# Arlo0o/StereoScene

Hardware: AMD Instinct MI355X
Metric: voxels/sec fwd+bwd, 256x256x32 grid D=192 (higher is better)
Workload: dtype f32; 1 GPU; kitti_d192: stereo pair features 2x[B,640,48,160] -> 256x256x32 occupancy, D=192, fwd+bwd incl. 4 losses; batch_per_gpu=1, global_batch=1, parallelism=dp1, train_mode=True

## Files before the change

### stereoscene_amd/csrc/conv_mfma.hip

```cpp
#include "common.h"
#include "conv_bf16.h"
#include "conv_thin_mfma.h"

#include <algorithm>
#include <cstdio>
#include <vector>
#include <array>
#include <map>
#include <mutex>
#include <type_traits>

namespace {

typedef float f32x16 __attribute__((ext_vector_type(16)));

struct ConvGeom {
  int B, Cin, Cout, CinPad, CoutPad;
  int Di, Hi, Wi, Do, Ho, Wo;
  int kd, kh, kw, sd, sh, sw, pd, ph, pw, dd, dh, dw;
  int form;
  int relu, accumulate;
  int hint;
  int chunk_taps;
  int bf16;
// ... 452 lines not shown
      if (khi >= g.kh || kwi >= g.kw) continue;
      const int tap = (kdi * g.kh + khi) * g.kw + kwi;
      float* dst = ws + (((size_t)chunk_id * taps + tap) * g.Cq) * g.Cp;
#pragma unroll
      for (int a = 0; a < MQ; ++a)
#pragma unroll
        for (int e = 0; e < MP; ++e)
#pragma unroll
          for (int r = 0; r < 16; ++r) {
            const int row = (qt * MQ + a) * 32 + (r & 3) + 8 * (r >> 2) + 4 * lk;
            if (row < g.Cq && pok[e]) dst[(size_t)row * g.Cp + poff[e]] = acc[a][e][c][t][r];
          }
    }
}

__global__ void __launch_bounds__(256)
wgrad_reduce_kernel(const float* __restrict__ ws, float* __restrict__ gw, int nchunks, int taps, int Cq, int Cp,
                    long total, long cstride) {
  __shared__ float part[8][33];
  const int e = threadIdx.x & 31, row = threadIdx.x >> 5;
  const long i = (long)blockIdx.x * 32 + e;
  float s = 0.0f;
  if (i < total)
    for (int c = row; c < nchunks; c += 8) s += ws[(size_t)c * cstride + i];
  part[row][e] = s;
  __syncthreads();
  if (row == 0 && i < total) {
    float t = 0.0f;
#pragma unroll
    for (int r = 0; r < 8; ++r) t += part[r][e];
    const int p = (int)(i % Cp);
    const int q = (int)((i / Cp) % Cq);
    const int tap = (int)(i / ((long)Cp * Cq));
    gw[((size_t)p * Cq + q) * taps + tap] = t;
  }
}

__global__ void __launch_bounds__(256)
wgrad_reduce_tiled_kernel(const float* __restrict__ ws, float* __restrict__ gw, int nchunks, int taps, int Cq, int Cp,
                          long total, long cstride) {
  extern __shared__ float tile[];
  const int P = 8 * taps + 1;
  const int e = threadIdx.x & 31, row = threadIdx.x >> 5;
  const int p0 = blockIdx.x * 32, q0 = blockIdx.y * 8;
  const bool ok = p0 + e < Cp && q0 + row < Cq;
  for (int tap = 0; tap < taps; ++tap) {
    float s = 0.0f;
    if (ok) {
      const float* src = ws + ((size_t)tap * Cq + q0 + row) * Cp + p0 + e;
#pragma unroll 4
      for (int c = 0; c < nchunks; ++c) s += src[(size_t)c * cstride];
    }
    tile[e * P + row * taps + tap] = s;
  }
  __syncthreads();
  const int run = 8 * taps;
  for (int j = threadIdx.x; j < 32 * run; j += 256) {
    const int pe = j / run, r = j - pe * run;
    const int q = q0 + r / taps, tap = r % taps, pp = p0 + pe;
    if (pp < Cp && q < Cq) gw[((size_t)pp * Cq + q) * taps + tap] = tile[pe * P + r];
  }
}

typedef float wr_f4 __attribute__((ext_vector_type(4)));
__global__ void __launch_bounds__(256)
wgrad_reduce_stage_kernel(float* __restrict__ ws, int nchunks, int per, long total4) {
  const long j = (long)blockIdx.x * 256 + threadIdx.x;
  if (j >= total4) return;
  const int c0 = blockIdx.y * per, c1 = min(nchunks, c0 + per);
  wr_f4* base = reinterpret_cast<wr_f4*>(ws) + (size_t)c0 * total4 + j;
  const wr_f4* p = base;
  wr_f4 a[8];
#pragma unroll
  for (int u = 0; u < 8; ++u) a[u] = wr_f4{0.0f, 0.0f, 0.0f, 0.0f};
  for (int c = c0; c < c1; c += 8) {
#pragma unroll
    for (int u = 0; u < 8; ++u)
      if (c + u < c1) a[u] += p[(size_t)u * total4];
    p += 8 * total4;
  }
  *base = ((a[0] + a[1]) + (a[2] + a[3])) + ((a[4] + a[5]) + (a[6] + a[7]));
}

void launch_wgrad_reduce(float* partial, float* gw, int nchunks, int taps, int Cq, int Cp, hipStream_t st) {
  const long total = (long)taps * Cq * Cp;
  long cstride = total;
  static const int two_stage = ssbev_tune("SSBEV_WGRAD_REDUCE2") ? atoi(ssbev_tune("SSBEV_WGRAD_REDUCE2")) : 1;
  if (two_stage && nchunks >= 64 && total % 4 == 0) {
    const long total4 = total / 4, bx = cdiv(total4, 256);
    int nsl = (int)std::min<long>(std::max<long>(cdiv(2048, bx), 1), nchunks / 8);
    const int per = cdiv(nchunks, nsl);
    nsl = cdiv(nchunks, per);
    hipLaunchKernelGGL(wgrad_reduce_stage_kernel, dim3((unsigned)bx, (unsigned)nsl), dim3(256), 0, st, partial, nchunks, per,
                       total4);
    nchunks = nsl;
    cstride = (long)per * total;
  }
  if (taps <= 32 && (long)cdiv(Cp, 32) * cdiv(Cq, 8) >= 128) {
    hipLaunchKernelGGL(wgrad_reduce_tiled_kernel, dim3(cdiv(Cp, 32), cdiv(Cq, 8)), dim3(256),
                       (size_t)32 * (8 * taps + 1) * sizeof(float), st, partial, gw, nchunks, taps, Cq, Cp, total, cstride);
  } else {
    hipLaunchKernelGGL(wgrad_reduce_kernel, dim3(cdiv(total, 32)), dim3(256), 0, st, partial, gw, nchunks, taps, Cq, Cp,
                       total, cstride);
  }
}

bool conv_dims_ok(const ssbev_conv_dims* d) {
  if (!d) return false;
  if (d->B <= 0 || d->Cin <= 0 || d->Cout <= 0) return false;
  if (d->Di <= 0 || d->Hi <= 0 || d->Wi <= 0 || d->Do <= 0 || d->Ho <= 0 || d->Wo <= 0) return false;
  if (d->kd <= 0 || d->kh <= 0 || d->kw <= 0 || d->sd <= 0 || d->sh <= 0 || d->sw <= 0) return false;
  if (d->dd <= 0 || d->dh <= 0 || d->dw <= 0 || d->pd < 0 || d->ph < 0 || d->pw < 0) return false;
  if (d->kd > 8 || d->kh > 8 || d->kw > 8) return false;
  const bool strided = d->sd > 1 || d->sh > 1 || d->sw > 1;
  const bool dilated = d->dd > 1 || d->dh > 1 || d->dw > 1;
  if (strided && dilated) return false;
  return true;
}

int pad8(int c) { return (c + 7) & ~7; }
int pad32(int c) { return (c + 31) & ~31; }
size_t align256b(size_t x) { return (x + 255) & ~(size_t)255; }

bool is_k3_p1_d1(const ssbev_conv_dims* d, int s) {
  return d->kd == 3 && d->kh == 3 && d->kw == 3 && d->sd == s && d->sh == s && d->sw == s &&
         d->pd == 1 && d->ph == 1 && d->pw == 1 && d->dd == 1 && d->dh == 1 && d->dw == 1;
}
bool same_grid(const ssbev_conv_dims* d) { return d->Di == d->Do && d->Hi == d->Ho && d->Wi == d->Wo; }

ConvGeom make_gather_geom(const ssbev_conv_dims* d, int mode) {
  const bool fwd = mode == 0;
  ConvGeom g;
  g.B = d->B; g.Cin = fwd ? d->Cin : d->Cout; g.Cout = fwd ? d->Cout : d->Cin; g.CinPad = pad8(g.Cin); g.CoutPad = pad32(g.Cout);
  g.Di = fwd ? d->Di : d->Do; g.Hi = fwd ? d->Hi : d->Ho; g.Wi = fwd ? d->Wi : d->Wo;
  g.Do = fwd ? d->Do : d->Di; g.Ho = fwd ? d->Ho : d->Hi; g.Wo = fwd ? d->Wo : d->Wi;
  g.kd = d->kd; g.kh = d->kh; g.kw = d->kw; g.sd = d->sd; g.sh = d->sh; g.sw = d->sw;
  g.pd = d->pd; g.ph = d->ph; g.pw = d->pw; g.dd = d->dd; g.dh = d->dh; g.dw = d->dw;
  g.form = (d->transposed != 0) == fwd ? 1 : 0;
  g.relu = fwd ? d->relu : 0; g.accumulate = d->accumulate;
  g.hint = d->tile_hint >= 10 ? d->tile_hint : 0;
  g.chunk_taps = 0; g.bf16 = d->precision == 1;
  return g;
}

template <int MT, int NT, int QU>
int launch_gather(const float* x, const float* wp, const float* bias, float* y, const ConvGeom& g, hipStream_t st) {
  long Mtot = (long)g.B * g.Do * g.Ho * g.Wo;
  int classes = 1;
  if (g.form == 1) {
    classes = g.sd * g.sh * g.sw;
    Mtot = (long)g.B * ((g.Do + g.sd - 1) / g.sd) * ((g.Ho + g.sh - 1) / g.sh) * ((g.Wo + g.sw - 1) / g.sw);
  }
  dim3 grid(cdiv(Mtot, 4 * MT * 32), cdiv(g.Cout, NT * 32), classes), block(256);
  constexpr bool PIPE = NT == 5;
  if (g.bf16) {
    constexpr int QB = QU < 2 ? 2 : QU;
    if ((g.CinPad >> 3) % QB == 0)
      hipLaunchKernelGGL((conv_gather_kernel<MT, NT, QB, 4, false, PIPE, true>), grid, block, 0, st, x, wp, bias, y, g);
    else if ((g.CinPad >> 3) % 2 == 0)
      hipLaunchKernelGGL((conv_gather_kernel<MT, NT, 2, 4, false, PIPE, true>), grid, block, 0, st, x, wp, bias, y, g);
    else
      hipLaunchKernelGGL((conv_gather_kernel<MT, NT, 1, 4, false, false, true>), grid, block, 0, st, x, wp, bias, y, g);
    return ssbev_launch_status();
  }
  if ((g.CinPad >> 3) % QU == 0)
    hipLaunchKernelGGL((conv_gather_kernel<MT, NT, QU, 4, false, PIPE>), grid, block, 0, st, x, wp, bias, y, g);
  else
    hipLaunchKernelGGL((conv_gather_kernel<MT, NT, 1, 4, false, PIPE>), grid, block, 0, st, x, wp, bias, y, g);
  return ssbev_launch_status();
}

template <int MT, int QU>
int launch_gather_ldsb(const float* x, const float* wp, const float* bias, float* y, const ConvGeom& g, hipStream_t st) {
  constexpr int WPB = 16;
  long Mtot = (long)g.B * g.Do * g.Ho * g.Wo;
  int classes = 1;
  if (g.form == 1) {
    classes = g.sd * g.sh * g.sw;
    Mtot = (long)g.B * ((g.Do + g.sd - 1) / g.sd) * ((g.Ho + g.sh - 1) / g.sh) * ((g.Wo + g.sw - 1) / g.sw);
  }
  const size_t per_tap = (size_t)(g.CinPad >> 3) * 2 * 32 * 16;
  const int taps_total = g.kd * g.kh * g.kw;
  int chunk = (int)((144 * 1024) / per_tap);
  if (chunk < 1) return SSBEV_EINVAL;
  if (chunk > taps_total) chunk = taps_total;
  const int passes = (taps_total + chunk - 1) / chunk;
  chunk = (taps_total + passes - 1) / passes;
  ConvGeom gg = g;
  gg.chunk_taps = chunk;
  const size_t lds = per_tap * chunk;
  auto kern = g.bf16 ? conv_gather_kernel<MT, 1, QU, WPB, true, false, true> : conv_gather_kernel<MT, 1, QU, WPB, true>;
  if (lds > 64 * 1024 && hipFuncSetAttribute(reinterpret_cast<const void*>(kern),
                                              hipFuncAttributeMaxDynamicSharedMemorySize, (int)lds) != hipSuccess)
    return SSBEV_ELAUNCH;
  dim3 grid(cdiv(Mtot, WPB * MT * 32), cdiv(g.Cout, 32), classes), block(WPB * 64);
  hipLaunchKernelGGL(kern, grid, block, lds, st, x, wp, bias, y, gg);
  return ssbev_launch_status();
}

template <int MT, int NT>
int launch_gather_qu(int qu, const float* x, const float* wp, const float* bias, float* y, const ConvGeom& g,
                     hipStream_t st) {
  if (qu == 4) return launch_gather<MT, NT, 4>(x, wp, bias, y, g, st);
  if (qu == 2) return launch_gather<MT, NT, 2>(x, wp, bias, y, g, st);
  return launch_gather<MT, NT, 1>(x, wp, bias, y, g, st);
}

int launch_gather_cfg(int mt, int nt, int qu, const float* x, const float* wp, const float* bias, float* y,
                      const ConvGeom& g, hipStream_t st) {
  switch (mt * 10 + nt) {
    case 41: return launch_gather_qu<4, 1>(qu, x, wp, bias, y, g, st);
    case 21: return launch_gather_qu<2, 1>(qu, x, wp, bias, y, g, st);
    case 11: return launch_gather_qu<1, 1>(qu, x, wp, bias, y, g, st);
    case 24: return launch_gather_qu<2, 4>(qu, x, wp, bias, y, g, st);
    case 22: return launch_gather_qu<2, 2>(qu, x, wp, bias, y, g, st);
    case 12: return launch_gather_qu<1, 2>(qu, x, wp, bias, y, g, st);
    case 15: return launch_gather_qu<1, 5>(qu, x, wp, bias, y, g, st);
    case 14: return launch_gather_qu<1, 4>(qu, x, wp, bias, y, g, st);
    case 31: return launch_gather_qu<3, 1>(qu, x, wp, bias, y, g, st);
    case 23: return launch_gather_qu<2, 3>(qu, x, wp, bias, y, g, st);
    case 26: return launch_gather_qu<2, 6>(qu, x, wp, bias, y, g, st);
    case 16: return launch_gather_qu<1, 6>(qu, x, wp, bias, y, g, st);
    case 13: return launch_gather_qu<1, 3>(qu, x, wp, bias, y, g, st);
    case 91: return launch_gather_ldsb<2, 2>(x, wp, bias, y, g, st);
    case 92: return launch_gather_ldsb<1, 2>(x, wp, bias, y, g, st);
    default: return SSBEV_EINVAL;
  }
}

long gather_blocks(const ConvGeom& g, int MT, int NT) {
  long M = (long)g.B * g.Do * g.Ho * g.Wo;
  long classes = 1;
  if (g.form == 1) {
    classes = (long)g.sd * g.sh * g.sw;
    M = (long)g.B * ((g.Do + g.sd - 1) / g.sd) * ((g.Ho + g.sh - 1) / g.sh) * ((g.Wo + g.sw - 1) / g.sw);
  }
  return ((M + 4 * MT * 32 - 1) / (4 * MT * 32)) * ((g.Cout + NT * 32 - 1) / (NT * 32)) * classes;
}

__device__ const float kGatherZeros[4] __attribute__((aligned(16))) = {0.f, 0.f, 0.f, 0.f};

template <int WN, int MW, int WGN>
__global__ void __launch_bounds__(256, 2)
conv_igemm_kernel(const float* __restrict__ x, const float* __restrict__ wp, const float* __restrict__ bias,
                  float* __restrict__ y, ConvGeom g, int mblocks, int nblocks) {
  constexpr int WGM = 4 / WGN;
  constexpr int BM = 32 * MW * WGM, BN = 32 * WN * WGN, BK = 32;
  constexpr int AF = BM * BK, BF = BK * BN, SF = AF + BF;
  constexpr int AI = AF / 256, BI = BF / 256;
  constexpr int AE = (AI + 3) / 4, BE = (BI + 3) / 4;
  extern __shared__ __align__(16) float lds[];
  long* t_src = reinterpret_cast<long*>(lds + 2 * SF);
  long* t_dst = t_src + BM;
  unsigned* t_msk = reinterpret_cast<unsigned*>(t_dst + BM);
  const int tid = threadIdx.x, lane = tid & 63, wave = __builtin_amdgcn_readfirstlane(tid >> 6);
  const int li = lane & 31, lk = lane >> 5;
  const int wm = wave / WGN, wn = wave % WGN;

  int par_d = 0, par_h = 0, par_w = 0;
  int Dc = g.Do, Hc = g.Ho, Wc = g.Wo;
  if (g.form == 1) {
    int cls = (int)gridDim.z - 1 - (int)blockIdx.z;
    par_w = cls % g.sw; cls /= g.sw;
    par_h = cls % g.sh; cls /= g.sh;
    par_d = cls;
    Dc = (g.Do - par_d + g.sd - 1) / g.sd; Hc = (g.Ho - par_h + g.sh - 1) / g.sh; Wc = (g.Wo - par_w + g.sw - 1) / g.sw;
  }
  const long Mtot = (long)g.B * Dc * Hc * Wc;
  int mb, nb;
  {
    const unsigned n = gridDim.x, L = blockIdx.x;
    const unsigned xcd = L & 7, q = n >> 3, r = n & 7;
    const unsigned base = xcd < r ? xcd * (q + 1) : r * (q + 1) + (xcd - r) * q;
    const unsigned Lp = base + (L >> 3);
    nb = (int)(Lp % (unsigned)nblocks);
    mb = (int)(Lp / (unsigned)nblocks);
  }
  const long m0 = (long)mb * BM;
  const int n0 = nb * BN;
  if (m0 >= Mtot) return;

  int kd0 = 0, kh0 = 0, kw0 = 0, kds = 1, khs = 1, kws = 1;
  if (g.form == 1) {
    kd0 = (par_d + g.pd) % g.sd; kh0 = (par_h + g.ph) % g.sh; kw0 = (par_w + g.pw) % g.sw;
    kds = g.sd; khs = g.sh; kws = g.sw;
  }
  const int nkd = (g.kd - kd0 + kds - 1) / kds, nkh = (g.kh - kh0 + khs - 1) / khs, nkw = (g.kw - kw0 + kws - 1) / kws;
  const int ntaps = (kd0 < g.kd && kh0 < g.kh && kw0 < g.kw) ? nkd * nkh * nkw : 0;
  int step_d, step_h, step_w;
  if (g.form == 0) { step_d = g.dd; step_h = g.dh; step_w = g.dw; }
  else { step_d = -(kds * g.dd) / g.sd; step_h = -(khs * g.dh) / g.sh; step_w = -(kws * g.dw) / g.sw; }

  if (tid < BM) {
    long m = m0 + tid;
    const bool ok = m < Mtot;
    if (!ok) m = 0;
    const int ow = (int)(m % Wc); m /= Wc;
    const int oh = (int)(m % Hc); m /= Hc;
    const int od = (int)(m % Dc);
    const int ob = (int)(m / Dc);
    int bd, bh, bw;
    if (g.form == 0) {
      bd = od * g.sd - g.pd; bh = oh * g.sh - g.ph; bw = ow * g.sw - g.pw;
    } else {
      bd = od + (par_d + g.pd - kd0 * g.dd) / g.sd;
      bh = oh + (par_h + g.ph - kh0 * g.dh) / g.sh;
      bw = ow + (par_w + g.pw - kw0 * g.dw) / g.sw;
    }
    unsigned msk = 0;
    for (int i = 0; i < nkd && i < 8; ++i) { const int v = bd + i * step_d; msk |= (v >= 0 && v < g.Di) ? (1u << i) : 0u; }
    for (int i = 0; i < nkh && i < 8; ++i) { const int v = bh + i * step_h; msk |= (v >= 0 && v < g.Hi) ? (1u << (8 + i)) : 0u; }
    for (int i = 0; i < nkw && i < 8; ++i) { const int v = bw + i * step_w; msk |= (v >= 0 && v < g.Wi) ? (1u << (16 + i)) : 0u; }
    t_msk[tid] = ok ? msk : 0u;
    t_src[tid] = ((((long)ob * g.Di + bd) * g.Hi + bh) * g.Wi + bw) * (long)g.Cin;
    long dst;
    if (g.form == 0) dst = (((long)ob * g.Do + od) * g.Ho + oh) * g.Wo + ow;
    else dst = (((long)ob * g.Do + (od * g.sd + par_d)) * g.Ho + (oh * g.sh + par_h)) * g.Wo + (ow * g.sw + par_w);
    t_dst[tid] = ok ? dst * (long)g.Cout : -1;
  }
  __syncthreads();

  const float* ap[AE]; unsigned am[AE];
#pragma unroll
  for (int e = 0; e < AE; ++e) {
    const int item = (wave + 4 * e) * 64 + lane, row = item >> 3, slot = item & 7;
    const bool on = wave + 4 * e < AI;
    ap[e] = x + (on ? t_src[row] : 0) + ((slot ^ ((row >> 1) & 7)) << 2);
    am[e] = on ? t_msk[row] : 0u;
  }
  const int Q = g.CinPad >> 3;
  long boff[BE];
#pragma unroll
  for (int e = 0; e < BE; ++e) {
    const int j = wave + 4 * e, f = j * 256 + 4 * lane;
    const int r8 = f / (BN * 4), col = f % (BN * 4);
    boff[e] = n0 + col / 4 < g.CoutPad ? (long)r8 * g.CoutPad * 4 + (long)n0 * 4 + col : -1;
  }
  const int cq_n = g.Cin >> 5;
  const int nst = ntaps * cq_n;
  int i_ia = 0, i_ib = 0, i_ic = 0, i_cq = 0;
  auto issue = [&](int buf) {
    const int tap = ((kd0 + i_ia * kds) * g.kh + (kh0 + i_ib * khs)) * g.kw + (kw0 + i_ic * kws);
    const long toff = (((long)i_ia * step_d * g.Hi + (long)i_ib * step_h) * g.Wi + (long)i_ic * step_w) * g.Cin + i_cq * 32;
    const unsigned need = (1u << i_ia) | (1u << (8 + i_ib)) | (1u << (16 + i_ic));
#pragma unroll
    for (int e = 0; e < AE; ++e) {
      if (AI % 4 != 0 && wave + 4 * e >= AI) break;
      const float* src = ((am[e] & need) == need) ? ap[e] + toff : kGatherZeros;
      __builtin_amdgcn_global_load_lds(src, lds + buf * SF + (wave + 4 * e) * 256, 16, 0, 0);
    }
    const float* wb = wp + ((size_t)tap * Q + 4 * i_cq) * 2 * g.CoutPad * 4;
#pragma unroll
    for (int e = 0; e < BE; ++e) {
      if (BI % 4 != 0 && wave + 4 * e >= BI) break;
      const float* bsrc = boff[e] >= 0 ? wb + boff[e] : kGatherZeros;
      __builtin_amdgcn_global_load_lds(bsrc, lds + buf * SF + AF + (wave + 4 * e) * 256, 16, 0, 0);
    }
    if (++i_cq == cq_n) {
      i_cq = 0;
      if (++i_ic == nkw) { i_ic = 0; if (++i_ib == nkh) { i_ib = 0; ++i_ia; } }
    }
  };

  f32x16 acc[MW][WN];
#pragma unroll
  for (int mt = 0; mt < MW; ++mt)
#pragma unroll
    for (int nt = 0; nt < WN; ++nt)
#pragma unroll
      for (int r = 0; r < 16; ++r) acc[mt][nt][r] = 0.0f;

  typedef float v4f __attribute__((ext_vector_type(4)));
  if (nst > 0) issue(0);
  for (int st = 0; st < nst; ++st) {
    const int buf = st & 1;
    asm volatile("s_waitcnt vmcnt(0)" ::: "memory");
    __builtin_amdgcn_s_barrier();
    if (st + 1 < nst) issue(buf ^ 1);
    const float* as = lds + buf * SF;
    const float* bs = as + AF;
    v4f ac[MW], bc[WN], an[MW], bn[WN];
    auto fetch = [&](int q, v4f (&a)[MW], v4f (&bf)[WN]) {
#pragma unroll
      for (int mt = 0; mt < MW; ++mt) {
        const int row = (wm * MW + mt) * 32 + li;
        a[mt] = *reinterpret_cast<const v4f*>(as + row * BK + (((2 * q + lk) ^ ((row >> 1) & 7)) << 2));
      }
#pragma unroll
      for (int nt = 0; nt < WN; ++nt)
        bf[nt] = *reinterpret_cast<const v4f*>(bs + ((2 * q + lk) * BN + (wn * WN + nt) * 32 + li) * 4);
    };
    fetch(0, ac, bc);
#pragma unroll
    for (int q = 0; q < BK / 8; ++q) {
      if (q + 1 < BK / 8) fetch(q + 1, an, bn);
      __builtin_amdgcn_sched_barrier(0);
#pragma unroll
      for (int t = 0; t < 4; ++t)
#pragma unroll
        for (int mt = 0; mt < MW; ++mt)
#pragma unroll
          for (int nt = 0; nt < WN; ++nt)
            acc[mt][nt] = __builtin_amdgcn_mfma_f32_32x32x2f32(ac[mt][t], bc[nt][t], acc[mt][nt], 0, 0, 0);
#pragma unroll
      for (int mt = 0; mt < MW; ++mt) ac[mt] = an[mt];
#pragma unroll
      for (int nt = 0; nt < WN; ++nt) bc[nt] = bn[nt];
    }
    asm volatile("s_waitcnt lgkmcnt(0)" ::: "memory");
  }

  float bv[WN];
#pragma unroll
  for (int nt = 0; nt < WN; ++nt) {
    const int co = min(n0 + (wn * WN + nt) * 32 + li, g.Cout - 1);
    bv[nt] = bias ? bias[co] : 0.0f;
  }
  long rowbase[MW][16];
#pragma unroll
  for (int mt = 0; mt < MW; ++mt)
#pragma unroll
    for (int r = 0; r < 16; ++r) rowbase[mt][r] = t_dst[(wm * MW + mt) * 32 + (r & 3) + 8 * (r >> 2) + 4 * lk];
  if (g.accumulate) {
#pragma unroll
    for (int mt = 0; mt < MW; ++mt)
#pragma unroll
      for (int r0 = 0; r0 < 16; r0 += 8) {
        float oldv[8][WN];
#pragma unroll
        for (int r = 0; r < 8; ++r)
#pragma unroll
          for (int nt = 0; nt < WN; ++nt) {
            const int co = n0 + (wn * WN + nt) * 32 + li;
            oldv[r][nt] = (rowbase[mt][r0 + r] >= 0 && co < g.Cout) ? y[rowbase[mt][r0 + r] + co] : 0.0f;
          }
#pragma unroll
        for (int r = 0; r < 8; ++r)
#pragma unroll
          for (int nt = 0; nt < WN; ++nt) acc[mt][nt][r0 + r] += oldv[r][nt];
      }
  }
#pragma unroll
  for (int nt = 0; nt < WN; ++nt) asm volatile("" : "+v"(bv[nt]));
#pragma unroll
  for (int nt = 0; nt < WN; ++nt) {
    const int co = n0 + (wn * WN + nt) * 32 + li;
    if (co >= g.Cout) continue;
#pragma unroll
    for (int mt = 0; mt < MW; ++mt)
#pragma unroll
      for (int r = 0; r < 16; ++r) {
        if (rowbase[mt][r] >= 0) {
          float v = acc[mt][nt][r] + bv[nt];
          if (g.relu) v = fmaxf(v, 0.0f);
          y[rowbase[mt][r] + co] = v;
        }
      }
  }
}

bool conv_igemm_applicable(const ConvGeom& g) {
  const char* env = ssbev_env("SSBEV_IGEMM");
  const int mode = env ? atoi(env) : 2;
  if (mode == 0 || g.bf16 || g.hint) return false;
  if (g.Cin % 32 != 0 || g.Cout % 4 != 0 || g.Cout < 64) return false;
  if (g.kd > 8 || g.kh > 8 || g.kw > 8) return false;
  const int taps = g.kd * g.kh * g.kw;
  if (taps == 1) return false;
  if (g.form == 0 && g.sd * g.sh * g.sw == 1 && mode != 2)
    return false;
  const long M = (long)g.B * g.Do * g.Ho * g.Wo;
  return M >= 2048;
}

template <int WN, int MW, int WGN>
int launch_igemm_t(const float* x, const float* wp, const float* bias, float* y, const ConvGeom& g, hipStream_t st) {
  constexpr int BM = 32 * MW * (4 / WGN), BN = 32 * WN * WGN;
  long Mtot = (long)g.B * g.Do * g.Ho * g.Wo;
  int classes = 1;
  if (g.form == 1) {
    classes = g.sd * g.sh * g.sw;
    Mtot = (long)g.B * ((g.Do + g.sd - 1) / g.sd) * ((g.Ho + g.sh - 1) / g.sh) * ((g.Wo + g.sw - 1) / g.sw);
  }
  const int mblocks = (int)((Mtot + BM - 1) / BM), nblocks = (g.Cout + BN - 1) / BN;
  const size_t lds = (size_t)2 * (BM * 32 + 32 * BN) * sizeof(float) + (size_t)BM * (2 * sizeof(long) + sizeof(unsigned));
  auto kern = conv_igemm_kernel<WN, MW, WGN>;
  if (hipFuncSetAttribute(reinterpret_cast<const void*>(kern), hipFuncAttributeMaxDynamicSharedMemorySize, (int)lds) != hipSuccess)
    return SSBEV_ELAUNCH;
  hipLaunchKernelGGL(kern, dim3((unsigned)(mblocks * nblocks), 1, classes), dim3(256), lds, st, x, wp, bias, y, g, mblocks, nblocks);
  return ssbev_launch_status();
}

int launch_igemm(const float* x, const float* wp, const float* bias, float* y, const ConvGeom& g, hipStream_t st) {
  long Mtot = (long)g.B * g.Do * g.Ho * g.Wo;
  long classes = 1;
  if (g.form == 1) {
    classes = (long)g.sd * g.sh * g.sw;
    Mtot = (long)g.B * ((g.Do + g.sd - 1) / g.sd) * ((g.Ho + g.sh - 1) / g.sh) * ((g.Wo + g.sw - 1) / g.sw);
  }
  const int force = ssbev_tune("SSBEV_IGEMM_TILE") ? atoi(ssbev_tune("SSBEV_IGEMM_TILE")) : 0;
  const bool wide = g.CoutPad % 128 == 0;
  const long need = g.form == 1 ? 1024 : 512;
  const int cand[3][2] = {{128, wide ? 128 : 64}, {64, wide ? 128 : 64}, {64, 64}};
  int bm = 64, bn = 64;
  for (int i = 0; i < 3; ++i) {
    const long blocks = ((Mtot + cand[i][0] - 1) / cand[i][0]) * ((g.Cout + cand[i][1] - 1) / cand[i][1]) * classes;
    if (blocks >= need) { bm = cand[i][0]; bn = cand[i][1]; break; }
  }
  if (force) { bm = force / 1000; bn = force % 1000; }
  if (bm == 128 && bn == 128) return launch_igemm_t<2, 2, 2>(x, wp, bias, y, g, st);
  if (bm == 128 && bn == 64) return launch_igemm_t<1, 2, 2>(x, wp, bias, y, g, st);
  if (bm == 64 && bn == 128) return launch_igemm_t<2, 1, 2>(x, wp, bias, y, g, st);
  if (bm == 64 && bn == 64) return launch_igemm_t<1, 1, 2>(x, wp, bias, y, g, st);
  return SSBEV_EINVAL;
}

int dispatch_gather(const float* x, const float* wp, const float* bias, float* y, const ConvGeom& g, hipStream_t st) {
  if (g.hint) return launch_gather_cfg(g.hint / 100, (g.hint / 10) % 10, g.hint % 10, x, wp, bias, y, g, st);
  const long Mtot = (long)g.B * g.Do * g.Ho * g.Wo;
  if (Mtot <= 8192 && g.Cout % 160 == 0 && g.Cout >= 640 && g.sd * g.sh * g.sw == 1)
    return launch_gather_cfg(1, 5, 4, x, wp, bias, y, g, st);
  {
    const long classes = g.form == 1 ? (long)g.sd * g.sh * g.sw : 1;
    const long keff = g.form == 1 ? (long)cdiv(g.kd, g.sd) * cdiv(g.kh, g.sh) * cdiv(g.kw, g.sw) * g.Cin
                                  : (long)g.kd * g.kh * g.kw * g.Cin;
    if (Mtot / classes <= 8192 && keff <= 8192 && g.Cout > 64)
      return launch_gather_cfg(1, 1, g.form == 1 ? 1 : 4, x, wp, bias, y, g, st);
  }
  {
    const size_t wbytes = (size_t)g.kd * g.kh * g.kw * (g.CinPad >> 3) * 2 * 32 * 16;
    if (g.Cout <= 32 && wbytes <= 144 * 1024 && wbytes >= 32 * 1024 && (g.CinPad >> 3) % 2 == 0 &&
        gather_blocks(g, 2, 1) >= 2048)
      return launch_gather_ldsb<2, 2>(x, wp, bias, y, g, st);
  }
  if (g.Cout % 192 == 0 && gather_blocks(g, 2, 6) >= 256) return launch_gather_cfg(2, 6, 4, x, wp, bias, y, g, st);
  int nt = (g.Cout % 128 == 0) ? 4 : (g.Cout > 32 ? 2 : 1);
  if (nt == 4 && gather_blocks(g, 2, 4) < 256) nt = 2;
  const int mt = gather_blocks(g, 2, nt) >= 160 ? 2 : 1;
  int qu = gather_blocks(g, mt, nt) < 512 ? 4 : (nt == 4 ? 4 : (nt == 2 ? 1 : 2));
  if (g.form == 1 && nt == 1 && gather_blocks(g, mt, nt) >= 512) qu = 1;
  if (g.form == 1 && g.sd * g.sh * g.sw > 1) {
    return launch_gather_cfg(1, nt > 2 ? 2 : nt, 1, x, wp, bias, y, g, st);
  }
  return launch_gather_cfg(mt, nt, qu, x, wp, bias, y, g, st);
}

struct WgradCfg { int MQ, MP, TH, TW; };

WgradCfg wgrad_cfg(int Cp, int Cq, int kh, int kw) {
  if (kh * kw == 1) return {2, 2, 1, 1};
  if (Cp > 32 && Cq > 32) return {2, 2, 1, 3};
  if (Cp <= 32 && Cq <= 32) return {1, 1, 3, 3};
  return {1, 1, 1, 3};
}

template <int V> using Int = std::integral_constant<int, V>;
template <typename F>
void with_wgrad_cfg(const WgradCfg& c, F f) {
  if (c.TH == 1 && c.TW == 1) f(Int<2>{}, Int<2>{}, Int<1>{}, Int<1>{});
  else if (c.MQ == 2) f(Int<2>{}, Int<2>{}, Int<1>{}, Int<3>{});
  else if (c.TH == 3) f(Int<1>{}, Int<1>{}, Int<3>{}, Int<3>{});
  else f(Int<1>{}, Int<1>{}, Int<1>{}, Int<3>{});
}

struct __attribute__((packed, aligned(4))) f4u { float x, y, z, w; };

__global__ void __launch_bounds__(256)
transpose_pad_kernel(const float* __restrict__ src, float* __restrict__ dst, int C, int B, int D, int H, int W,
                     int pd, int ph, int pw, int Dp, int Hp, int Wp) {
  __shared__ float tile[32][65];
  const long V = (long)B * D * H * W;
  const long v0 = (long)blockIdx.x * 64;
  const int c0 = blockIdx.y * 32;
  for (int i = threadIdx.x; i < 64 * 8; i += 256) {
    const int r = i >> 3, c4 = (i & 7) * 4;
    const long v = v0 + r;
    float4 t = make_float4(0, 0, 0, 0);
    if (v < V && c0 + c4 < C) t = *reinterpret_cast<const float4*>(src + (size_t)v * C + c0 + c4);
    tile[c4 + 0][r] = t.x; tile[c4 + 1][r] = t.y; tile[c4 + 2][r] = t.z; tile[c4 + 3][r] = t.w;
  }
  __syncthreads();
  for (int i = threadIdx.x; i < 32 * 64; i += 256) {
    const int c = i >> 6, r = i & 63;
    const long v = v0 + r;
    if (v >= V || c0 + c >= C) continue;
    long t = v;
    const int w = (int)(t % W); t /= W;
    const int h = (int)(t % H); t /= H;
    const int d = (int)(t % D);
    const int b = (int)(t / D);
    dst[((((size_t)b * Dp + d + pd) * Hp + h + ph) * C + c0 + c) * Wp + w + pw] = tile[c][r];
  }
}

struct WgradCfGeom {
  int B, Cp, Cq, D, H, W;
  int kd, kh, kw, dd, dh, dw;
// ... 2792 lines not shown
  WgradDhPlan dh;
  WgradLdsPlan lds;
  WgradCfGeom cf;
  WgradGeom direct;
  WgradCfg cfg;
};

WgradPlan select_wgrad(const ssbev_conv_dims* d) {
  WgradPlan p{};
  const size_t tile = (size_t)d->Cin * d->Cout * sizeof(float);
  const size_t taps = (size_t)d->kd * d->kh * d->kw;
  if (ssbev_bf16::storage_mode(d)) {
    p.kind = WgradKind::Bf16Storage;
    p.ws_bytes = ssbev_bf16::wgrad_workspace(d);
  } else if (ssbev_thin::wgrad_applicable(d)) {
    p.kind = WgradKind::ThinSide;
    p.ws_bytes = ssbev_thin::wgrad_workspace(d);
  } else if ((p.thin = plan_wgrad_thin(d)).ok) {
    p.kind = WgradKind::Thin;
    p.ws_bytes = align256b((size_t)p.thin.nchunks * 27 * tile);
  } else if ((p.p1 = plan_wgrad_1x1(d)).ok && d->tile_hint != 7) {
    p.kind = WgradKind::Pointwise;
    p.ws_bytes = align256b(p.p1.nchunks * tile);
  } else if ((p.dh = plan_wgrad_dh(d)).ok) {
    p.kind = WgradKind::Dh;
    p.gu_off = align256b((size_t)p.dh.nchunks * 48 * tile);
    p.ws_bytes = p.gu_off + align256b(48 * tile);
  } else if ((p.lds = plan_wgrad_lds(d)).ok && d->tile_hint != 7) {
    p.kind = WgradKind::Lds;
    p.ws_bytes = align256b((size_t)p.lds.nchunks * p.lds.ksplit * d->kd * 9 * tile);
  } else if (wgrad_cf_applicable(d)) {
    p.kind = WgradKind::ChannelsFirst;
    const WgradCfGeom& g = p.cf = make_wgrad_cf_geom(d, &p.cfg);
    p.pt_off = align256b(g.nchunks * taps * tile);
    p.qp_off = p.pt_off + align256b((size_t)g.Cp * g.B * g.D * g.H * g.W * sizeof(float));
    p.qp_bytes = ((size_t)g.Cq * g.B * g.Dp * g.Hp * g.Wp + 16) * sizeof(float);
    p.ws_bytes = p.qp_off + align256b(p.qp_bytes);
  } else {
    p.kind = WgradKind::Direct;
    p.direct = make_wgrad_geom(d);
    p.cfg = wgrad_cfg(p.direct.Cp, p.direct.Cq, p.direct.kh, p.direct.kw);
    p.ws_bytes = p.direct.nchunks * taps * tile;
  }
  return p;
}

}

namespace ssbev_detail {
void wgrad_reduce(float* partial, float* gw, int nchunks, int taps, int Cq, int Cp, hipStream_t st) {
  launch_wgrad_reduce(partial, gw, nchunks, taps, Cq, Cp, st);
}
}

extern "C" {

int ssbev_conv_kernel_class(const ssbev_conv_dims* d, int mode) {
  if (!conv_dims_ok(d) || mode < 0 || mode > 2) return SSBEV_EINVAL;
  if (ssbev_bf16::storage_mode(d)) return ssbev_bf16::dims_ok(d, mode) ? ssbev_bf16::kernel_class(d, mode) : SSBEV_EINVAL;
  if (mode == 2) return ssbev_thin::wgrad_applicable(d) ? 6 : 0;
  const ConvPath path = select_conv_path(d, mode);
  if (path != ConvPath::ThinIn && ssbev_thin::thinout_applicable(d, mode)) return 5;
  return conv_path_class(path);
}

int ssbev_conv_chunk_groups(const ssbev_conv_dims* d, int mode) {
  if (!conv_dims_ok(d) || mode < 0 || mode > 2) return 0;
  if (mode == 2) {
    const WgradPlan p = select_wgrad(d);
    return p.kind == WgradKind::Dh ? p.dh.g.gpc : 0;
  }
  switch (ssbev_conv_kernel_class(d, mode)) {
    case 1: return plan_conv_tap(d, mode).gpc;
    case 2: return plan_conv_taph(d, mode).gpc;
    case 3: return plan_conv_thin(d, mode).gpc;
    case 7: return plan_conv_tap2(d, mode).gpc;
    case 8: return plan_conv_tap2up(d, mode).gpc;
    case 9: return plan_conv_tapdh(d, mode).gpc;
    case 17: return ssbev_bf16::tap_chunk_groups(d, mode);
    default: return 0;
  }
}

int ssbev_conv_bf16_plan_query(const ssbev_conv_dims* d, int mode, ssbev_conv_bf16_plan* out) {
  if (!conv_dims_ok(d) || !ssbev_bf16::storage_mode(d)) return SSBEV_EINVAL;
  return ssbev_bf16::plan_query(d, mode, out);
}

size_t ssbev_conv_packed_weight_elems(const ssbev_conv_dims* d) {
  if (!conv_dims_ok(d)) return 0;
  if (ssbev_bf16::storage_mode(d)) return ssbev_bf16::packed_elems(d);
  const size_t taps = (size_t)d->kd * d->kh * d->kw;
  const size_t a = (size_t)pad8(d->Cin) * pad32(d->Cout), b = (size_t)pad8(d->Cout) * pad32(d->Cin);
  const size_t generic = taps * (a > b ? a : b);
  const size_t special = (size_t)std::max(std::max(kTwPackedElems, kDhPackedElems), std::max(kT2PackedElems, kUpPackedElems));
  return generic > special ? generic : special;
}

int ssbev_conv_pack_weight(const float* w_src, float* w_packed, const ssbev_conv_dims* d, int mode,
                           ssbev_stream_t stream) {
  if (!conv_dims_ok(d) || !w_src || !w_packed || (mode != 0 && mode != 1)) return SSBEV_EINVAL;
  hipStream_t st = as_stream(stream);
  if (ssbev_bf16::storage_mode(d)) return ssbev_bf16::pack(w_src, w_packed, d, mode, st);
  const int K = mode == 0 ? d->Cin : d->Cout, N = mode == 0 ? d->Cout : d->Cin;
  const dim3 block(256);
  switch (select_conv_path(d, mode)) {
    case ConvPath::ThinIn: return ssbev_thin::thinin_pack(w_src, w_packed, d, mode, st);
    case ConvPath::Thin:
      hipLaunchKernelGGL(pack_thin_kernel, dim3(cdiv(27 * kThinNP * 32, 256)), block, 0, st, w_src, w_packed, d->Cout, d->Cin, mode);
      break;
    case ConvPath::Tap2:
      hipLaunchKernelGGL(pack_tap2_kernel, dim3(cdiv(kT2PackedElems, 256)), block, 0, st, w_src, w_packed, N, K);
      break;
    case ConvPath::Tap2Up:
      hipLaunchKernelGGL(pack_tap2up_kernel, dim3(cdiv(kUpPackedElems, 256)), block, 0, st, w_src, w_packed, N, K);
      break;
    case ConvPath::Pw32:
      hipLaunchKernelGGL(pack_pw32_kernel, dim3(cdiv(kPwPackedElems, 256)), block, 0, st, w_src, w_packed, d->Cout, d->Cin, mode);
      break;
    case ConvPath::TapDh:
      hipLaunchKernelGGL(pack_tapdh_kernel, dim3(cdiv(kDhPackedElems, 256)), block, 0, st, w_src, w_packed, d->Cout, d->Cin, mode);
      break;
    case ConvPath::TapH:
      hipLaunchKernelGGL(pack_taph_kernel, dim3(cdiv(kTwPackedElems, 256)), block, 0, st, w_src, w_packed, d->Cout, d->Cin, mode);
      break;
    case ConvPath::Tap:
      hipLaunchKernelGGL(pack_tap_kernel, dim3(cdiv(kTapPackedElems, 256)), block, 0, st, w_src, w_packed, d->Cout, d->Cin, mode);
      break;
    case ConvPath::Igemm: case ConvPath::Gather: case ConvPath::Invalid: {
      const int taps = d->kd * d->kh * d->kw;
      const int layout = (mode == 0) == (d->transposed == 0) ? 0 : 1;
      const int KPad = pad8(K), NPad = pad32(N);
      const long total = (long)taps * KPad * NPad;
      hipLaunchKernelGGL(pack_weight_kernel, dim3(cdiv(total, 256)), block, 0, st, w_src, w_packed, K, N, KPad, NPad, taps, layout,
                         total);
    }
  }
  return ssbev_launch_status();
}

int ssbev_conv_fwd_bf16(const uint16_t* x, const float* w_packed, const float* bias, void* y, const ssbev_conv_dims* d,
                        ssbev_stream_t stream) {
  if (!conv_dims_ok(d) || !ssbev_bf16::storage_mode(d) || !x || !w_packed || !y) return SSBEV_EINVAL;
  return ssbev_bf16::forward(x, w_packed, bias, y, d, as_stream(stream));
}

int ssbev_conv_bwd_data_bf16(const uint16_t* gy, const float* w_packed_t, void* gx, const ssbev_conv_dims* d,
                             ssbev_stream_t stream) {
  if (!conv_dims_ok(d) || !ssbev_bf16::storage_mode(d) || !gy || !w_packed_t || !gx) return SSBEV_EINVAL;
  return ssbev_bf16::backward_data(gy, w_packed_t, gx, d, as_stream(stream));
}

int ssbev_conv_bwd_weight_bf16(const uint16_t* x, const uint16_t* gy, float* gw, const ssbev_conv_dims* d, void* ws,
                               size_t ws_bytes, ssbev_stream_t stream) {
  if (!conv_dims_ok(d) || d->precision != 2 || !x || !gy || !gw || !ws) return SSBEV_EINVAL;
  return ssbev_bf16::backward_weight(x, gy, gw, d, ws, ws_bytes, as_stream(stream));
}

int ssbev_conv_fwd(const float* x, const float* w_packed, const float* bias, float* y,
                   const ssbev_conv_dims* d, ssbev_stream_t stream) {
  if (!conv_dims_ok(d) || !x || !w_packed || !y) return SSBEV_EINVAL;
  if (ssbev_bf16::storage_mode(d)) return SSBEV_EINVAL;
  return run_conv(x, w_packed, bias, y, d, 0, as_stream(stream));
}

int ssbev_conv_bwd_data(const float* gy, const float* w_packed_t, float* gx,
// ... 74 lines not shown
```

Measured before the change: 31.20 million voxels/s.

## Add three-stage LDS pipeline and one-round tile plans to implicit-GEMM conv

Templates the implicit-GEMM conv kernel on pipeline depth, adding a triple-buffered LDS path that waits with a counted vmcnt so one stage of global-to-LDS copies stays in flight while the current one is consumed. The tile planner now uses a 128x64 tile with three stages for strided form-1 convs with wide Cout. It also adds a 96x128 (or 64x128) tile for stride-1 convs when that gives roughly one wave of blocks. The extra LDS per stage may lower occupancy, and the new tiles change wave utilisation for those shapes.

```diff
diff --git a/stereoscene_amd/csrc/conv_mfma.hip b/stereoscene_amd/csrc/conv_mfma.hip
--- a/stereoscene_amd/csrc/conv_mfma.hip
+++ b/stereoscene_amd/csrc/conv_mfma.hip
@@ -716,7 +716,7 @@
 
 __device__ const float kGatherZeros[4] __attribute__((aligned(16))) = {0.f, 0.f, 0.f, 0.f};
 
-template <int WN, int MW, int WGN>
+template <int WN, int MW, int WGN, int NST = 2>
 __global__ void __launch_bounds__(256, 2)
 conv_igemm_kernel(const float* __restrict__ x, const float* __restrict__ wp, const float* __restrict__ bias,
                   float* __restrict__ y, ConvGeom g, int mblocks, int nblocks) {
@@ -725,8 +725,10 @@
   constexpr int AF = BM * BK, BF = BK * BN, SF = AF + BF;
   constexpr int AI = AF / 256, BI = BF / 256;
   constexpr int AE = (AI + 3) / 4, BE = (BI + 3) / 4;
+  constexpr int NG = (AI + BI) / 4;
+  static_assert(NST == 2 || (NST == 3 && AI % 4 == 0 && BI % 4 == 0), "conv_igemm_kernel: a counted wait needs the same copies in every wave");
   extern __shared__ __align__(16) float lds[];
-  long* t_src = reinterpret_cast<long*>(lds + 2 * SF);
+  long* t_src = reinterpret_cast<long*>(lds + NST * SF);
   long* t_dst = t_src + BM;
   unsigned* t_msk = reinterpret_cast<unsigned*>(t_dst + BM);
   const int tid = threadIdx.x, lane = tid & 63, wave = __builtin_amdgcn_readfirstlane(tid >> 6);
@@ -848,11 +850,13 @@
 
   typedef float v4f __attribute__((ext_vector_type(4)));
   if (nst > 0) issue(0);
-  for (int st = 0; st < nst; ++st) {
-    const int buf = st & 1;
-    asm volatile("s_waitcnt vmcnt(0)" ::: "memory");
+  if (NST == 3 && nst > 1) issue(1);
+  int buf = 0;
+  for (int st = 0; st < nst; ++st, buf = buf + 1 == NST ? 0 : buf + 1) {
+    if (NST == 3 && st + 1 < nst) asm volatile("s_waitcnt vmcnt(%0)" ::"n"(NG) : "memory");
+    else asm volatile("s_waitcnt vmcnt(0)" ::: "memory");
     __builtin_amdgcn_s_barrier();
-    if (st + 1 < nst) issue(buf ^ 1);
+    if (st + NST - 1 < nst) issue(buf == 0 ? NST - 1 : buf - 1);
     const float* as = lds + buf * SF;
     const float* bs = as + AF;
     v4f ac[MW], bc[WN], an[MW], bn[WN];
@@ -949,7 +953,7 @@
   return M >= 2048;
 }
 
-template <int WN, int MW, int WGN>
+template <int WN, int MW, int WGN, int NST>
 int launch_igemm_t(const float* x, const float* wp, const float* bias, float* y, const ConvGeom& g, hipStream_t st) {
   constexpr int BM = 32 * MW * (4 / WGN), BN = 32 * WN * WGN;
   long Mtot = (long)g.B * g.Do * g.Ho * g.Wo;
@@ -959,36 +963,60 @@
     Mtot = (long)g.B * ((g.Do + g.sd - 1) / g.sd) * ((g.Ho + g.sh - 1) / g.sh) * ((g.Wo + g.sw - 1) / g.sw);
   }
   const int mblocks = (int)((Mtot + BM - 1) / BM), nblocks = (g.Cout + BN - 1) / BN;
-  const size_t lds = (size_t)2 * (BM * 32 + 32 * BN) * sizeof(float) + (size_t)BM * (2 * sizeof(long) + sizeof(unsigned));
-  auto kern = conv_igemm_kernel<WN, MW, WGN>;
+  const size_t lds = (size_t)NST * (BM * 32 + 32 * BN) * sizeof(float) + (size_t)BM * (2 * sizeof(long) + sizeof(unsigned));
+  auto kern = conv_igemm_kernel<WN, MW, WGN, NST>;
   if (hipFuncSetAttribute(reinterpret_cast<const void*>(kern), hipFuncAttributeMaxDynamicSharedMemorySize, (int)lds) != hipSuccess)
     return SSBEV_ELAUNCH;
   hipLaunchKernelGGL(kern, dim3((unsigned)(mblocks * nblocks), 1, classes), dim3(256), lds, st, x, wp, bias, y, g, mblocks, nblocks);
   return ssbev_launch_status();
 }
 
-int launch_igemm(const float* x, const float* wp, const float* bias, float* y, const ConvGeom& g, hipStream_t st) {
+struct IgemmPlan { int bm, bn, nst; };
+
+IgemmPlan plan_igemm(const ConvGeom& g) {
   long Mtot = (long)g.B * g.Do * g.Ho * g.Wo;
   long classes = 1;
   if (g.form == 1) {
     classes = (long)g.sd * g.sh * g.sw;
     Mtot = (long)g.B * ((g.Do + g.sd - 1) / g.sd) * ((g.Ho + g.sh - 1) / g.sh) * ((g.Wo + g.sw - 1) / g.sw);
   }
-  const int force = ssbev_tune("SSBEV_IGEMM_TILE") ? atoi(ssbev_tune("SSBEV_IGEMM_TILE")) : 0;
   const bool wide = g.CoutPad % 128 == 0;
   const long need = g.form == 1 ? 1024 : 512;
-  const int cand[3][2] = {{128, wide ? 128 : 64}, {64, wide ? 128 : 64}, {64, 64}};
-  int bm = 64, bn = 64;
-  for (int i = 0; i < 3; ++i) {
-    const long blocks = ((Mtot + cand[i][0] - 1) / cand[i][0]) * ((g.Cout + cand[i][1] - 1) / cand[i][1]) * classes;
-    if (blocks >= need) { bm = cand[i][0]; bn = cand[i][1]; break; }
-  }
-  if (force) { bm = force / 1000; bn = force % 1000; }
-  if (bm == 128 && bn == 128) return launch_igemm_t<2, 2, 2>(x, wp, bias, y, g, st);
-  if (bm == 128 && bn == 64) return launch_igemm_t<1, 2, 2>(x, wp, bias, y, g, st);
-  if (bm == 64 && bn == 128) return launch_igemm_t<2, 1, 2>(x, wp, bias, y, g, st);
-  if (bm == 64 && bn == 64) return launch_igemm_t<1, 1, 2>(x, wp, bias, y, g, st);
-  return SSBEV_EINVAL;
+  const auto blocks_of = [&](int bm, int bn) { return ((Mtot + bm - 1) / bm) * ((g.Cout + bn - 1) / bn) * classes; };
+  const int cand[3][3] = {{128, wide ? 128 : 64, 2}, {g.form == 1 && wide ? 128 : 64, g.form == 1 || !wide ? 64 : 128, g.form == 1 && wide ? 3 : 2},
+                          {64, 64, 2}};
+  IgemmPlan p = {64, 64, 2};
+  for (int i = 0; i < 3; ++i)
+    if (blocks_of(cand[i][0], cand[i][1]) >= need) { p = {cand[i][0], cand[i][1], cand[i][2]}; break; }
+  if (g.form == 0 && wide) {
+    const int one_round[2][2] = {{96, 128}, {64, 128}};
+    for (int i = 0; i < 2; ++i) {
+      const long blocks = blocks_of(one_round[i][0], one_round[i][1]);
+      if (blocks >= 192 && blocks <= 256) { p = {one_round[i][0], one_round[i][1], 2}; break; }
+    }
+  }
+  if (const char* e = ssbev_tune("SSBEV_IGEMM_TILE")) { const int v = atoi(e); if (v > 0) { p.bm = v / 1000; p.bn = v % 1000; } }
+  if (const char* e = ssbev_tune("SSBEV_IGEMM_STAGES")) { const int v = atoi(e); if (v > 0) p.nst = v; }
+  return p;
+}
+
+int launch_igemm(const float* x, const float* wp, const float* bias, float* y, const ConvGeom& g, hipStream_t st) {
+  const IgemmPlan p = plan_igemm(g);
+  switch (p.bm * 10000 + p.bn * 10 + p.nst) {
+    case 1281282: return launch_igemm_t<2, 2, 2, 2>(x, wp, bias, y, g, st);
+    case 1280642: return launch_igemm_t<1, 2, 2, 2>(x, wp, bias, y, g, st);
+    case 641282: return launch_igemm_t<2, 1, 2, 2>(x, wp, bias, y, g, st);
+    case 640642: return launch_igemm_t<1, 1, 2, 2>(x, wp, bias, y, g, st);
+    case 1280643: return launch_igemm_t<1, 2, 2, 3>(x, wp, bias, y, g, st);
+    case 961282: return launch_igemm_t<1, 3, 4, 2>(x, wp, bias, y, g, st);
+#ifdef SSBEV_TUNING
+    case 641283: return launch_igemm_t<2, 1, 2, 3>(x, wp, bias, y, g, st);
+    case 640643: return launch_igemm_t<1, 1, 2, 3>(x, wp, bias, y, g, st);
+    case 1281283: return launch_igemm_t<2, 2, 2, 3>(x, wp, bias, y, g, st);
+    case 961283: return launch_igemm_t<1, 3, 4, 3>(x, wp, bias, y, g, st);
+#endif
+    default: return SSBEV_EINVAL;
+  }
 }
 
 int dispatch_gather(const float* x, const float* wp, const float* bias, float* y, const ConvGeom& g, hipStream_t st) {
@@ -3947,6 +3975,12 @@
   }
 }
 
+int ssbev_conv_igemm_tile(const ssbev_conv_dims* d, int mode) {
+  if (!conv_dims_ok(d) || mode < 0 || mode > 1 || ssbev_conv_kernel_class(d, mode) != 11) return 0;
+  const IgemmPlan p = plan_igemm(make_gather_geom(d, mode));
+  return p.bm * 10000 + p.bn * 10 + p.nst;
+}
+
 int ssbev_conv_bf16_plan_query(const ssbev_conv_dims* d, int mode, ssbev_conv_bf16_plan* out) {
   if (!conv_dims_ok(d) || !ssbev_bf16::storage_mode(d)) return SSBEV_EINVAL;
   return ssbev_bf16::plan_query(d, mode, out);
```

Result: no change. 31.19 million voxels/s (-0.0%).

## Fuse two-stage wgrad partial reduction into a single kernel for untiled shapes

Applied to the files above, without the earlier changes.

Adds a fused weight-gradient reduce kernel. Each block handles 32 float4 columns, and its 8 rows of threads each sum over a subset of chunk slices. The partial sums are combined in shared memory and written straight into the transposed gw layout. This removes the second launch and the intermediate global write and read of the stage-1 slice results. In exchange, each block has less parallelism per column, and the final store to gw is scattered.

```diff
diff --git a/stereoscene_amd/csrc/conv_mfma.hip b/stereoscene_amd/csrc/conv_mfma.hip
--- a/stereoscene_amd/csrc/conv_mfma.hip
+++ b/stereoscene_amd/csrc/conv_mfma.hip
@@ -558,21 +558,70 @@
   *base = ((a[0] + a[1]) + (a[2] + a[3])) + ((a[4] + a[5]) + (a[6] + a[7]));
 }
 
+__global__ void __launch_bounds__(256)
+wgrad_reduce_fused_kernel(const float* __restrict__ ws, float* __restrict__ gw, int nchunks, int per, int nsl, int taps, int Cq,
+                          int Cp, long total4) {
+  __shared__ float part[8][128];
+  const int e = threadIdx.x & 31, row = threadIdx.x >> 5;
+  const long j = (long)blockIdx.x * 32 + e;
+  const wr_f4 zero = wr_f4{0.0f, 0.0f, 0.0f, 0.0f};
+  auto slice = [&](int y) {
+    const int c0 = y * per, c1 = y < nsl ? min(nchunks, c0 + per) : c0;
+    const wr_f4* p = reinterpret_cast<const wr_f4*>(ws) + (size_t)c0 * total4 + j;
+    wr_f4 a[8];
+#pragma unroll
+    for (int u = 0; u < 8; ++u) a[u] = zero;
+    for (int c = c0; c < c1; c += 8) {
+#pragma unroll
+      for (int u = 0; u < 8; ++u)
+        if (c + u < c1) a[u] += p[(size_t)u * total4];
+      p += 8 * total4;
+    }
+    return ((a[0] + a[1]) + (a[2] + a[3])) + ((a[4] + a[5]) + (a[6] + a[7]));
+  };
+  wr_f4 s = zero;
+  if (j < total4)
+    for (int y = row; y < nsl; y += 16) {
+      const wr_f4 s0 = slice(y), s1 = slice(y + 8);
+      s += s0;
+      if (y + 8 < nsl) s += s1;
+    }
+#pragma unroll
+  for (int k = 0; k < 4; ++k) part[row][4 * e + k] = s[k];
+  __syncthreads();
+  const long i = (long)blockIdx.x * 128 + threadIdx.x;
+  if (threadIdx.x < 128 && i < 4 * total4) {
+    float t = 0.0f;
+#pragma unroll
+    for (int r = 0; r < 8; ++r) t += part[r][threadIdx.x];
+    const int p = (int)(i % Cp);
+    const int q = (int)((i / Cp) % Cq);
+    const int tap = (int)(i / ((long)Cp * Cq));
+    gw[((size_t)p * Cq + q) * taps + tap] = t;
+  }
+}
+
 void launch_wgrad_reduce(float* partial, float* gw, int nchunks, int taps, int Cq, int Cp, hipStream_t st) {
   const long total = (long)taps * Cq * Cp;
   long cstride = total;
+  const bool tiled = taps <= 32 && (long)cdiv(Cp, 32) * cdiv(Cq, 8) >= 128;
   static const int two_stage = ssbev_tune("SSBEV_WGRAD_REDUCE2") ? atoi(ssbev_tune("SSBEV_WGRAD_REDUCE2")) : 1;
   if (two_stage && nchunks >= 64 && total % 4 == 0) {
     const long total4 = total / 4, bx = cdiv(total4, 256);
     int nsl = (int)std::min<long>(std::max<long>(cdiv(2048, bx), 1), nchunks / 8);
     const int per = cdiv(nchunks, nsl);
     nsl = cdiv(nchunks, per);
+    if (!tiled && two_stage != 2) {
+      hipLaunchKernelGGL(wgrad_reduce_fused_kernel, dim3((unsigned)cdiv(total4, 32)), dim3(256), 0, st, partial, gw, nchunks, per,
+                         nsl, taps, Cq, Cp, total4);
+      return;
+    }
     hipLaunchKernelGGL(wgrad_reduce_stage_kernel, dim3((unsigned)bx, (unsigned)nsl), dim3(256), 0, st, partial, nchunks, per,
                        total4);
     nchunks = nsl;
     cstride = (long)per * total;
   }
-  if (taps <= 32 && (long)cdiv(Cp, 32) * cdiv(Cq, 8) >= 128) {
+  if (tiled) {
     hipLaunchKernelGGL(wgrad_reduce_tiled_kernel, dim3(cdiv(Cp, 32), cdiv(Cq, 8)), dim3(256),
                        (size_t)32 * (8 * taps + 1) * sizeof(float), st, partial, gw, nchunks, taps, Cq, Cp, total, cstride);
   } else {
```

New measurement: 31.08 million voxels/s before, 31.19 million voxels/s after, median of 6. No clear change (+0.4%).
